# ViliamVadocz/takzero

Measured on AMD Instinct MI355X. Metric: mcts_simulations_per_s, higher is better.
Workload: dtype f16

## Files before the change

takzero_amd/build.py:

```python
import os
import subprocess
import sys

HERE = os.path.dirname(os.path.abspath(__file__))
CSRC = os.path.join(HERE, "csrc")
OUT = os.path.join(HERE, "libtakzero_hip.so")
ARCH = "gfx950"
UNITS = [
    ("tz_text.cpp", ["-ffp-contract=off"]),
    ("tz_ot.cpp", []),
    ("tz_host.cpp", ["-ffp-contract=off"]),
    ("tz_host_learn.cpp", ["-ffp-contract=off"]),
    ("tz_comm.cpp", []),
    ("tz_tree.hip", ["-ffp-contract=off", "-fhip-fp32-correctly-rounded-divide-sqrt"]),
    ("tz_capi.hip", ["-ffp-contract=off", "-fhip-fp32-correctly-rounded-divide-sqrt"]),
    ("tz_nn.hip", []),
    ("tz_nn_split.hip", []),
    ("tz_nn_c6.hip", []),
    ("tz_nn_c6b.hip", []),
    ("tz_nn_c6c.hip", []),
    ("tz_learn.hip", ["-ffp-contract=off"]),
]
COMMON = ["-O3", "-std=c++17", "-fPIC", "--offload-arch=" + ARCH, "-fno-fast-math", "-Wall", "-Wno-unused-function",
          "-Wno-unused-result"]


def _stale(target, deps):
    if not os.path.exists(target):
        return True
    t = os.path.getmtime(target)
    return any(os.path.getmtime(d) > t for d in deps)


def build(force=False, verbose=False, ablations=None):
    hipcc = os.environ.get("HIPCC", "/opt/rocm/bin/hipcc")
    if ablations is None:
        ablations = os.environ.get("TZ_BUILD_ABLATIONS", "0") not in ("", "0")
    stamp = os.path.join(CSRC, ".ablations")
    if ablations != os.path.exists(stamp):
        force_nn = True
        if ablations:
            open(stamp, "w").close()
        elif os.path.exists(stamp):
            os.remove(stamp)
    else:
        force_nn = False
    headers = [os.path.join(CSRC, f) for f in os.listdir(CSRC) if f.endswith(".h")]
    headers.append(os.path.join(os.path.dirname(HERE), "include", "takzero_hip.h"))
    objs = []
    procs = []
    for src, extra in UNITS:
        s = os.path.join(CSRC, src)
        o = os.path.join(CSRC, src.rsplit(".", 1)[0] + ".o")
        objs.append(o)
        nn = src in ("tz_nn.hip", "tz_nn_split.hip", "tz_nn_c6.hip", "tz_nn_c6b.hip", "tz_nn_c6c.hip")
        deps = [s] + headers + ([os.path.join(CSRC, "tz_nn.hip")] if nn else []) + ([os.path.join(CSRC, "tz_nn_c6.hip")] if src.startswith("tz_nn_c6") else [])
        if force or _stale(o, deps) or (force_nn and nn):
            cmd = [hipcc] + COMMON + extra + (["-DTZ_ABLATIONS"] if ablations and nn else []) + ["-x", "hip", "-c", s, "-o", o]
            if verbose:
                print(" ".join(cmd))
            procs.append((src, subprocess.Popen(cmd, stdout=subprocess.PIPE, stderr=subprocess.STDOUT)))
    failed = False
    for src, p in procs:
        out, _ = p.communicate()
        if p.returncode != 0:
            failed = True
            sys.stderr.write("---- %s ----\n%s\n" % (src, out.decode(errors="replace")))
        elif verbose and out:
            sys.stderr.write(out.decode(errors="replace"))
    if failed:
        raise RuntimeError("hipcc failed")
    if force or procs or _stale(OUT, objs):
        cmd = [hipcc, "-shared", "-fPIC", "--offload-arch=" + ARCH, "-o", OUT] + objs + ["-ldl"]
        subprocess.check_call(cmd)
    return OUT


if __name__ == "__main__":
    print(build(force="--force" in sys.argv, verbose=True, ablations=True if "--ablations" in sys.argv else None))
```

takzero_amd/csrc/tz_nn.hip:

```cpp
#include "tz_nn.h"
#include "tz_fp8.h"
#include "tz_fp6.h"
#include <type_traits>
#include "tz_ot.h"

#include <algorithm>
#include <cmath>
#include <cstdio>
#include <cstdlib>
#include <cstring>
#include <atomic>
#include <map>
#include <memory>
#include <mutex>
#include <thread>

int tz_nn_launch_split(int sp, int n, const void* net_args, int max_positions, hipStream_t st);
int tz_nn_launch_c6(int n, const void* net_args, int max_positions, hipStream_t st);
size_t tz_nn_c6_seed_bytes(int n, int max_positions);

namespace {

typedef float f32x4 __attribute__((ext_vector_type(4)));
typedef unsigned int u32x4 __attribute__((ext_vector_type(4)));
typedef __bf16 bf16x8 __attribute__((ext_vector_type(8)));
typedef __bf16 bf16x4 __attribute__((ext_vector_type(4)));
typedef _Float16 f16x8 __attribute__((ext_vector_type(8)));
typedef _Float16 f16x4 __attribute__((ext_vector_type(4)));

template <typename ET>
struct Elem;
template <>
struct Elem<__bf16> {
    typedef bf16x8 x8;
    typedef bf16x4 x4;
    static __device__ __forceinline__ f32x4 mfma(x8 a, x8 b, f32x4 c) { return __builtin_amdgcn_mfma_f32_16x16x32_bf16(a, b, c, 0, 0, 0); }
    static __device__ __forceinline__ __bf16 cvt(float x) { return (__bf16)x; }
    static __device__ __forceinline__ __bf16 relu_cvt(float x) { return (__bf16)(x > 0.f ? x : 0.f); }
};
template <>
struct Elem<_Float16> {
    typedef f16x8 x8;
    typedef f16x4 x4;
    static __device__ __forceinline__ f32x4 mfma(x8 a, x8 b, f32x4 c) { return __builtin_amdgcn_mfma_f32_16x16x32_f16(a, b, c, 0, 0, 0); }
    static __device__ __forceinline__ _Float16 cvt(float x) { return (_Float16)__builtin_amdgcn_fmed3f(x, -65504.0f, 65504.0f); }
    static __device__ __forceinline__ _Float16 relu_cvt(float x) { return (_Float16)__builtin_amdgcn_fmed3f(x, 0.0f, 65504.0f); }
};


constexpr int LDS_ROWB = 64;
constexpr int FILTERS = 256;
__device__ __forceinline__ int lds_piece(int row, int q) { return ((q + 2 * ((row >> 2) & 1)) & 3) << 4; }
template <int LAYOUT>
struct LdsImg {
    static constexpr int ROW_PAD = 528;
    __host__ __device__ static constexpr size_t bytes(int lrows) { return LAYOUT ? (size_t)lrows * LDS_ROWB * 8 : (size_t)lrows * ROW_PAD; }
    __device__ static __forceinline__ int store_addr(int row, int ci, int plane_bytes) {
        return LAYOUT ? (ci >> 2) * plane_bytes + row * LDS_ROWB + lds_piece(row, ci & 3) : row * ROW_PAD + ci * 16;
    }
    __device__ static __forceinline__ int read_base(bool ok, int v, int q, int zrow) {
        if (LAYOUT) {
            const int sr = ok ? v : zrow + (v & 7);
            return sr * LDS_ROWB + lds_piece(sr, q);
        }
        return (ok ? v : zrow) * ROW_PAD + q * 16;
    }
};

__host__ __device__ constexpr int c6_position_of(int c) {
    const int w = c >> 5, o = c & 31;
    return 32 * (4 * (w >> 2) + (o >> 3)) + 8 * (w & 3) + (o & 7);
}
__host__ __device__ constexpr int c6_channel_at(int pos) {
    const int plane = pos >> 5, piece = (pos >> 3) & 3, e = pos & 7;
    return 32 * (4 * (plane >> 2) + piece) + 8 * (plane & 3) + e;
}
static_assert(c6_channel_at(c6_position_of(77)) == 77 && c6_position_of(c6_channel_at(200)) == 200 && c6_position_of(32) == 8 && c6_position_of(8) == 32, "c6 channel places");

__host__ __device__ constexpr int ppt_for(int nb) { return nb == 1 ? 64 : nb == 3 ? 16 : nb == 4 ? 12 : nb == 5 ? 8 : 4; }

__device__ __forceinline__ void default_reserves_d(int n, int& stones, int& caps) {
    stones = n == 3 ? 10 : n == 4 ? 15 : n == 5 ? 21 : 30;
    caps = n >= 5 ? 1 : 0;
}

template <int NB>
__device__ __forceinline__ float plane_value(const tz_state* s, int px, int c, int flat_diff) {
    constexpr int SS = 3 + (NB - 1) + (NB + 1), NN = NB * NB;
    const int to_move = s->to_move;
    if (c < 2 * SS) {
        const int side = c / SS, k = c % SS;
        const int top = s->top[px], h = s->height[px];
        if (top == TZ_EMPTY) return 0.0f;
        const unsigned long long colors = s->colors[px];
        if (k < 3) {
            const int topc = (int)((colors >> (h - 1)) & 1ull);
            return (top == k + 1 && (topc != to_move) == (side == 1)) ? 1.0f : 0.0f;
        }
        const int idx = h - 2 - (k - 3);
        if (idx < 0) return 0.0f;
        const int color = (int)((colors >> idx) & 1ull);
        return ((color != to_move) == (side == 1)) ? 1.0f : 0.0f;
    }
    const int e = c - 2 * SS;
    int ds, dc;
    default_reserves_d(NB, ds, dc);
    const int mine = to_move, other = 1 - to_move;
    switch (e) {
        case 0: return (float)s->stones[mine] / (float)ds;
        case 1: return dc ? (float)s->caps[mine] / (float)dc : 0.0f;
        case 2: return (float)s->stones[other] / (float)ds;
        case 3: return dc ? (float)s->caps[other] / (float)dc : 0.0f;
        case 4: return to_move == 1 ? 1.0f : 0.0f;
        case 5: return ((float)flat_diff - (float)s->half_komi / 2.0f) / (float)NN;
        default: return 0.0f;
    }
}

template <int NB>
__device__ __forceinline__ int state_flat_diff(const tz_state* s) {
    int d = 0;
    for (int i = 0; i < NB * NB; i++) {
        if (s->top[i] == TZ_FLAT) {
            const int col = (int)((s->colors[i] >> (s->height[i] - 1)) & 1ull);
            d += col == 0 ? 1 : -1;
        }
    }
    return d;
}

struct ConvArgs {
    const void* in;
    const tz_state* states;
    const int32_t* game_index;
    const int32_t* count_dev;
    int count_host;
    const uint16_t* w;
    const float* bias;
    const void* residual;
    void* out;
    int cin_pad, kc_total, ct_total, out_stride, cin_real;
    int relu, out_f32, has_res;
    int in_stride;
    int groups;
    int in_z, w_z_frags, bias_z, out_z;
};

template <int NB, int RT, int TAPS, int LAYOUT>
__device__ __forceinline__ void tap_bases(const int (&yx)[RT], int tap, int lr, int q, int zrow, int (&abase)[RT]) {
    const int dy = TAPS == 9 ? tap / 3 - 1 : 0, dx = TAPS == 9 ? tap % 3 - 1 : 0;
#pragma unroll
    for (int rt = 0; rt < RT; rt++) {
        const int y = (yx[rt] & 0xff) + dy, x = (yx[rt] >> 8) + dx;
        const bool ok = y >= 0 && y < NB && x >= 0 && x < NB;
        abase[rt] = LdsImg<LAYOUT>::read_base(ok, rt * 16 + lr + dy * NB + dx, q, zrow);
    }
}

template <int NB, int RT, int TAPS, int LAYOUT>
__device__ __forceinline__ void tap_bases_rc(int tap, int lr, int q, int rows, int zrow, int (&abase)[RT]) {
    constexpr int NN = NB * NB;
    const int dy = TAPS == 9 ? tap / 3 - 1 : 0, dx = TAPS == 9 ? tap % 3 - 1 : 0;
#pragma unroll
    for (int rt = 0; rt < RT; rt++) {
        const int r = rt * 16 + lr, px = r % NN;
        const int y = px / NB + dy, x = px % NB + dx;
        const bool ok = r < rows && y >= 0 && y < NB && x >= 0 && x < NB;
        abase[rt] = LdsImg<LAYOUT>::read_base(ok, r + dy * NB + dx, q, zrow);
    }
}

template <int NB, int P, int RN, int TAPS, bool FROM_STATE, int ABL = 0, bool SINGLE = false, int NW = 8, int LAYOUT = 1, typename ET = __bf16, int OCC = 2>
__global__ __launch_bounds__(NW * 64, OCC) void conv_mfma_kernel(ConvArgs a) {
    typedef typename Elem<ET>::x8 ex8;
    typedef typename Elem<ET>::x4 ex4;
    constexpr int NT = NW * 64;
    constexpr int NN = NB * NB, ROWS = P * NN, RT = (ROWS + 15) / 16, LROWS = RT * 16 + 8, ZROW = RT * 16;
    constexpr int PLANE = LROWS * LDS_ROWB;
    constexpr int KSTEP = LAYOUT ? PLANE : 64;
    extern __shared__ __attribute__((aligned(16))) unsigned char lds[];
    const int count = a.count_dev ? *a.count_dev : a.count_host;
    const int pos0 = blockIdx.x * P;
    if (pos0 >= count) return;
    const int tid = threadIdx.x, lane = tid & 63;
    const int wave = __builtin_amdgcn_readfirstlane(tid >> 6);
    const int q = lane >> 4, lr = lane & 15;
    const int valid_rows = min(ROWS, (count - pos0) * NN);
    const size_t m0 = (size_t)pos0 * NN;
    const int ct0 = (blockIdx.y * NW + wave) * RN;
    const __amdgpu_buffer_rsrc_t wrsrc = __builtin_amdgcn_make_buffer_rsrc(
        const_cast<uint16_t*>(a.w), 0, (a.groups > 1 ? a.groups * a.w_z_frags : TAPS * a.kc_total * a.ct_total) * 1024, 0x00020000);
    const int lane16 = lane * 16;
    auto wload = [&](int tap, int kcg, int j) -> ex8 {
        const int frag = (int)blockIdx.z * a.w_z_frags + (tap * a.kc_total + kcg) * a.ct_total + (ct0 + j);
        const u32x4 r = __builtin_amdgcn_raw_buffer_load_b128(wrsrc, lane16, frag * 1024, 0);
        return __builtin_bit_cast(ex8, r);
    };
    f32x4 acc[RT][RN];

    if constexpr (SINGLE) {
        static_assert(!FROM_STATE, "SINGLE is for bf16 activations");
        {
            const uint16_t* in = reinterpret_cast<const uint16_t*>(a.in);
            constexpr int NLOAD = (LROWS * 32 + NT - 1) / NT;
            uint4 v[NLOAD];
#pragma unroll
            for (int i = 0; i < NLOAD; i++) {
                const int id = tid + i * NT, row = id >> 5, ci = id & 31;
                v[i] = make_uint4(0, 0, 0, 0);
                if (row < valid_rows) v[i] = *reinterpret_cast<const uint4*>(in + (m0 + row) * 256 + ci * 8);
            }
#pragma unroll
            for (int i = 0; i < NLOAD; i++) {
                const int id = tid + i * NT, row = id >> 5, ci = id & 31;
                if (row < LROWS) *reinterpret_cast<uint4*>(lds + LdsImg<LAYOUT>::store_addr(row, ci, PLANE)) = v[i];
            }
        }
        ex8 bq[4][RN];
#pragma unroll
        for (int j = 0; j < RN; j++) {
            bq[0][j] = wload(0, 0, j);
            bq[1][j] = wload(0, 1, j);
        }
        __syncthreads();
#pragma unroll
        for (int rt = 0; rt < RT; rt++)
#pragma unroll
            for (int j = 0; j < RN; j++) acc[rt][j] = f32x4{0.f, 0.f, 0.f, 0.f};
        int abase[RT];
        tap_bases_rc<NB, RT, TAPS, LAYOUT>(0, lr, q, ROWS, ZROW, abase);
        ex8 av[RT];
#pragma unroll
        for (int rt = 0; rt < RT; rt++) av[rt] = *reinterpret_cast<const ex8*>(lds + abase[rt]);
        for (int tap = 0; tap < TAPS; tap++) {
#pragma unroll
            for (int kc = 0; kc < 8; kc++) {
                if constexpr ((ABL & 2) == 0) {
                    if (kc + 2 < 8) {
#pragma unroll
                        for (int j = 0; j < RN; j++) bq[(kc + 2) & 3][j] = wload(tap, kc + 2, j);
                    } else if (tap + 1 < TAPS) {
#pragma unroll
                        for (int j = 0; j < RN; j++) bq[(kc + 2) & 3][j] = wload(tap + 1, kc + 2 - 8, j);
                    }
                    __builtin_amdgcn_sched_barrier(0);
                }
                if (kc == 7) {
                    int lr_t = lr;
                    asm volatile("" : "+v"(lr_t));
                    tap_bases_rc<NB, RT, TAPS, LAYOUT>(tap + 1 < TAPS ? tap + 1 : tap, lr_t, q, ROWS, ZROW, abase);
                }
                if (LAYOUT == 1 && kc == 4) {
#pragma unroll
                    for (int rt = 0; rt < RT; rt++) {
                        abase[rt] += 4 * PLANE;
                        asm volatile("" : "+v"(abase[rt]));
                    }
                }
#pragma unroll
                for (int rt = 0; rt < RT; rt++) {
#pragma unroll
                    for (int j = 0; j < RN; j++)
                        acc[rt][j] = Elem<ET>::mfma(bq[kc & 3][j], av[rt], acc[rt][j]);
                    if constexpr ((ABL & 1) == 0) {
                        if (kc < 7) av[rt] = *reinterpret_cast<const ex8*>(lds + abase[rt] + (kc + 1 - (LAYOUT == 1 && kc >= 4 ? 4 : 0)) * KSTEP);
                        else av[rt] = *reinterpret_cast<const ex8*>(lds + abase[rt]);
                    }
                }
            }
        }
    } else {
        int yx[RT];
#pragma unroll
        for (int rt = 0; rt < RT; rt++) {
            const int r = rt * 16 + lr, px = r % NN;
            yx[rt] = r < ROWS ? ((px / NB) | ((px % NB) << 8)) : 0x7f7f;
        }
#pragma unroll
        for (int rt = 0; rt < RT; rt++)
#pragma unroll
            for (int j = 0; j < RN; j++) acc[rt][j] = f32x4{0.f, 0.f, 0.f, 0.f};
        const int nslices = (a.cin_pad + 255) / 256;
        constexpr int NLOAD = FROM_STATE ? 1 : (LROWS * 32 + NT - 1) / NT;
        uint4 stage[NLOAD];
        auto fetch_slice = [&](int slice) {
            const int cpr_s = min(256, a.cin_pad - slice * 256) / 8;
            const uint16_t* in = reinterpret_cast<const uint16_t*>(a.in) + (size_t)blockIdx.z * a.in_z + slice * 256;
#pragma unroll
            for (int i = 0; i < NLOAD; i++) {
                const int id = tid + i * NT, row = id >> 5, ci = id & 31;
                stage[i] = make_uint4(0, 0, 0, 0);
                if (row < valid_rows && ci < cpr_s) stage[i] = *reinterpret_cast<const uint4*>(in + (m0 + row) * a.in_stride + ci * 8);
            }
        };
        if constexpr (!FROM_STATE) fetch_slice(0);
        for (int slice = 0; slice < nslices; slice++) {
            const int cs = min(256, a.cin_pad - slice * 256);
            const int kcs = cs / 32, cpr = cs / 8;
            __syncthreads();
            if constexpr (FROM_STATE) {
                for (int row = tid; row < LROWS; row += NT) {
                    const bool ok = row < valid_rows;
                    const tz_state* s = nullptr;
                    int px = 0, fd = 0;
                    if (ok) {
                        const int pos = pos0 + row / NN;
                        px = row % NN;
                        s = a.states + (a.game_index ? a.game_index[pos] : pos);
                        fd = state_flat_diff<NB>(s);
                    }
                    for (int c8 = 0; c8 < cpr; c8++) {
                        ex8 v;
#pragma unroll
                        for (int k = 0; k < 8; k++) {
                            const int c = c8 * 8 + k;
                            v[k] = (ET)((ok && c < a.cin_real) ? plane_value<NB>(s, px, c, fd) : 0.0f);
                        }
                        *reinterpret_cast<ex8*>(lds + LdsImg<LAYOUT>::store_addr(row, c8, PLANE)) = v;
                    }
                }
            } else {
#pragma unroll
// ... 2328 lines not shown
                                p8[at] = tz_f32_to_e4m3((wv - (float)hi) * 2048.0f * sw);
                                p8[at + 64 * 32] = tz_f32_to_e4m3((float)hi * sw);
                            }
                        }
            if ((rc = upload(p8, &L->w8))) return rc;
        }
        if (with_c6) {
            if (L->cin_pad % 128) return tz_fail(TZ_EINVAL, "weights: TZ_PREC_F16C6 needs input channels in multiples of 128");
            const int g_total = L->cin_pad / 128;
            constexpr size_t REC = 3328;
            std::vector<unsigned char> p6((size_t)taps * g_total * ct_total * REC, 0);
            for (int t = 0; t < taps; t++)
                for (int g = 0; g < g_total; g++)
                    for (int ct = 0; ct < ct_total; ct++) {
                        unsigned char* rec = p6.data() + (((size_t)t * g_total + g) * ct_total + ct) * REC;
                        for (int lane = 0; lane < 64; lane++) {
                            const int co = ct * 16 + (lane & 15), q = lane >> 4;
                            float lo[32], hi[32], amax_l = 0.0f, amax_h = 0.0f;
                            for (int i = 0; i < 32; i++) {
                                const int ci = 128 * g + 32 * (i >> 3) + 8 * q + (i & 7);
                                const float wv = (co < cout && ci < cin) ? W(co, ci, t) : 0.0f;
                                const _Float16 h = (_Float16)wv;
                                hi[i] = (float)h;
                                lo[i] = wv - (float)h;
                                amax_h = std::max(amax_h, fabsf(hi[i]));
                                amax_l = std::max(amax_l, fabsf(lo[i]));
                            }
                            const uint32_t bl = tz_e2m3_block_scale_byte(amax_l), bh = tz_e2m3_block_scale_byte(amax_h);
                            uint8_t cl[32], ch[32];
                            for (int i = 0; i < 32; i++) {
                                cl[i] = tz_f32_to_e2m3(ldexpf(lo[i], 127 - (int)bl));
                                ch[i] = tz_f32_to_e2m3(ldexpf(hi[i], 127 - (int)bh));
                            }
                            uint32_t sl[6], sh[6];
                            tz_pack_fp6x32(cl, sl);
                            tz_pack_fp6x32(ch, sh);
                            memcpy(rec + 0 * 1536 + lane * 16, sl, 16);
                            memcpy(rec + 0 * 1536 + 1024 + lane * 8, sl + 4, 8);
                            memcpy(rec + 1 * 1536 + lane * 16, sh, 16);
                            memcpy(rec + 1 * 1536 + 1024 + lane * 8, sh + 4, 8);
                            const uint32_t sw = bl | (bh << 8);
                            memcpy(rec + 3072 + lane * 4, &sw, 4);
                        }
                    }
            if ((rc = upload(p6, &L->w8))) return rc;
        }
        return upload(p, &L->w_mfma);
    }
    std::vector<float> f((size_t)taps * cin * cout);
    for (int t = 0; t < taps; t++)
        for (int ci = 0; ci < cin; ci++)
            for (int co = 0; co < cout; co++) f[((size_t)t * cin + ci) * cout + co] = W(co, ci, t);
    return upload(f, &L->w_f32);
}

void free_layer(ConvW* L) {
    if (L->w_mfma) (void)hipFree(L->w_mfma);
    if (L->w_lo) (void)hipFree(L->w_lo);
    if (L->w8) (void)hipFree(L->w8);
    if (L->w_f32) (void)hipFree(L->w_f32);
    if (L->bias) (void)hipFree(L->bias);
    *L = ConvW();
}

int bn_fold(const TensorMap& m, const std::string& p, int c, std::vector<float>& scale, std::vector<float>& bias) {
    std::vector<float> g, b, mean, var;
    int rc;
    if ((rc = get_tensor(m, p + ".weight", c, g))) return rc;
    if ((rc = get_tensor(m, p + ".bias", c, b))) return rc;
    if ((rc = get_tensor(m, p + ".running_mean", c, mean))) return rc;
    if ((rc = get_tensor(m, p + ".running_var", c, var))) return rc;
    scale.resize(c);
    bias.resize(c);
    for (int i = 0; i < c; i++) {
        const float s = g[i] / sqrtf(var[i] + 1e-5f);
        scale[i] = s;
        bias[i] = b[i] - mean[i] * s;
    }
    return TZ_OK;
}

struct NetWeights {
    ConvW conv_in, policy;
    std::vector<ConvW> res;
    uint16_t* tower_w = nullptr;
    uint16_t* tower_w_lo = nullptr;
    unsigned char* tower_w8 = nullptr;
    float* c8_scales = nullptr;
    float* tower_bias = nullptr;
    float* heads = nullptr;
    ConvW rnd[2][3];
    uint16_t* rndw[3] = {nullptr, nullptr, nullptr};
    float* rndb[3] = {nullptr, nullptr, nullptr};
    float rnd_min = 0.f, rnd_max = 1.f;
    float* simhash = nullptr;
};

void free_weights(NetWeights& w) {
    free_layer(&w.conv_in);
    free_layer(&w.policy);
    for (auto& l : w.res) free_layer(&l);
    w.res.clear();
    if (w.tower_w) (void)hipFree(w.tower_w);
    if (w.tower_w_lo) (void)hipFree(w.tower_w_lo);
    if (w.tower_w8) (void)hipFree(w.tower_w8);
    if (w.c8_scales) (void)hipFree(w.c8_scales);
    if (w.tower_bias) (void)hipFree(w.tower_bias);
    w.tower_w = nullptr;
    w.tower_w_lo = nullptr;
    w.tower_w8 = nullptr;
    w.c8_scales = nullptr;
    w.tower_bias = nullptr;
    if (w.heads) (void)hipFree(w.heads);
    w.heads = nullptr;
    for (int a = 0; a < 2; a++)
        for (int b = 0; b < 3; b++) free_layer(&w.rnd[a][b]);
    for (int l = 0; l < 3; l++) {
        if (w.rndw[l]) (void)hipFree(w.rndw[l]);
        if (w.rndb[l]) (void)hipFree(w.rndb[l]);
        w.rndw[l] = nullptr;
        w.rndb[l] = nullptr;
    }
    if (w.simhash) (void)hipFree(w.simhash);
    w.simhash = nullptr;
}

int build_weights(tz_net* net, const TensorMap& m, NetWeights& W) {
    const int nn = net->nn, cin = net->cin, prec = net->precision;
    std::vector<float> w, scale, bias;
    int rc;
    if ((rc = get_tensor(m, "core.input_conv2d.weight", (size_t)FILTERS * cin * 9, w))) return rc;
    if ((rc = bn_fold(m, "core.batch_norm", FILTERS, scale, bias))) return rc;
    const bool split = prec == TZ_PREC_F16X2, c8 = prec == TZ_PREC_F16C8, c6 = prec == TZ_PREC_F16C6;
    std::vector<int> c6_perm(FILTERS);
    for (int pos = 0; pos < FILTERS; pos++) c6_perm[pos] = c6_channel_at(pos);
    const std::vector<int>* tower_perm = c6 ? &c6_perm : nullptr;
    if ((rc = build_layer(prec, 9, cin, FILTERS, 256, w, scale, bias, nullptr, &W.conv_in, split || c8 || c6))) return rc;
    W.res.resize(2 * net->blocks);
    {
        const int nl = 2 * net->blocks;
        const int workers = std::max(1, std::min(nl, std::min(16, (int)std::thread::hardware_concurrency())));
        std::atomic<int> next{0}, failed{TZ_OK};
        std::string first_error;
        std::mutex mu;
        const bool background = g_upload_stream != nullptr;
        auto work = [&]() {
            if (hipSetDevice(net->device) != hipSuccess) {
                failed = TZ_EDEVICE;
                return;
            }
            std::unique_ptr<UploadStream> upload_stream(background ? new UploadStream() : nullptr);
            if (upload_stream && !upload_stream->mine) {
                std::lock_guard<std::mutex> lk(mu);
                if (failed == TZ_OK) {
                    failed = TZ_EDEVICE;
                    first_error = "weights: cannot create an upload stream for a build thread";
                }
                return;
            }
            std::vector<float> lw, lscale, lbias;
            for (int l = next++; l < nl && failed == TZ_OK; l = next++) {
                const std::string p = "core.res_block_" + std::to_string(l / 2) + ((l & 1) ? ".b" : ".a");
                int r = get_tensor(m, p + ".conv2d.weight", (size_t)FILTERS * FILTERS * 9, lw);
                if (!r) r = bn_fold(m, p + ".batch_norm", FILTERS, lscale, lbias);
                if (!r) r = build_layer(prec, 9, FILTERS, FILTERS, 256, lw, lscale, lbias, tower_perm, &W.res[l], split, c8, c6);
                if (r) {
                    std::lock_guard<std::mutex> lk(mu);
                    if (failed == TZ_OK) {
                        failed = r;
                        first_error = tz_last_error();
                    }
                }
            }
        };
        std::vector<std::thread> pool;
        for (int t = 1; t < workers; t++) pool.emplace_back(work);
        work();
        for (auto& t : pool) t.join();
        if (failed != TZ_OK) return tz_fail(failed, first_error.empty() ? "weights: a tower layer could not be built" : first_error);
    }
    if (prec != TZ_PREC_F32 && net->blocks > 0) {
        const size_t layer_elems = (size_t)9 * 8 * 16 * 64 * 8, nl = W.res.size();
        TZ_HIP(hipMalloc(&W.tower_w, nl * layer_elems * 2));
        if (split) TZ_HIP(hipMalloc(&W.tower_w_lo, nl * layer_elems * 2));
        const size_t layer_bytes8 = c6 ? (size_t)9 * 2 * 16 * 3328 : (size_t)9 * 2 * 16 * 2 * 64 * 32;
        if (c8 || c6) TZ_HIP(hipMalloc(&W.tower_w8, nl * layer_bytes8));
        TZ_HIP(hipMalloc(&W.tower_bias, nl * FILTERS * sizeof(float)));
        for (size_t l = 0; l < nl; l++) {
            if ((rc = copy_sync(W.tower_w + l * layer_elems, W.res[l].w_mfma, layer_elems * 2, hipMemcpyDeviceToDevice))) return rc;
            if (split && (rc = copy_sync(W.tower_w_lo + l * layer_elems, W.res[l].w_lo, layer_elems * 2, hipMemcpyDeviceToDevice))) return rc;
            if ((c8 || c6) && (rc = copy_sync(W.tower_w8 + l * layer_bytes8, W.res[l].w8, layer_bytes8, hipMemcpyDeviceToDevice))) return rc;
            if ((rc = copy_sync(W.tower_bias + l * FILTERS, W.res[l].bias, FILTERS * sizeof(float), hipMemcpyDeviceToDevice))) return rc;
        }
    }
    if ((rc = get_tensor(m, "policy.conv2d.weight", (size_t)net->pol_ch * FILTERS * 9, w))) return rc;
    if ((rc = get_tensor(m, "policy.conv2d.bias", net->pol_ch, bias))) return rc;
    if ((rc = build_layer(prec, 9, FILTERS, net->pol_ch, net->pol_stride, w, {}, bias, tower_perm, &W.policy, split, c8, c6))) return rc;
    if (c8) {
        std::vector<float> cs;
        for (auto& l : W.res) cs.push_back(l.c8_scale);
        cs.push_back(W.policy.c8_scale);
        if ((rc = upload(cs, &W.c8_scales))) return rc;
    }
    std::vector<float> hv, hu, lv, lu, t1;
    if ((rc = get_tensor(m, "value.conv2d.weight", FILTERS, hv))) return rc;
    if ((rc = get_tensor(m, "ube.conv2d.weight", FILTERS, hu))) return rc;
    if ((rc = get_tensor(m, "value.linear.weight", nn, lv))) return rc;
    if ((rc = get_tensor(m, "ube.linear.weight", nn, lu))) return rc;
    std::vector<float> hw;
    hw.insert(hw.end(), hv.begin(), hv.end());
    hw.insert(hw.end(), hu.begin(), hu.end());
    hw.insert(hw.end(), lv.begin(), lv.end());
    hw.insert(hw.end(), lu.begin(), lu.end());
    for (const char* nm : {"value.conv2d.bias", "ube.conv2d.bias", "value.linear.bias", "ube.linear.bias"}) {
        if ((rc = get_tensor(m, nm, 1, t1))) return rc;
        hw.push_back(t1[0]);
    }
    if ((rc = upload(hw, &W.heads))) return rc;
    if (net->has_rnd) {
        const int in_size = cin * nn;
        std::vector<int> perm(in_size);
        for (int px = 0; px < nn; px++)
            for (int c = 0; c < cin; c++) perm[px * cin + c] = c * nn + px;
        const char* nets[2] = {"rnd_learning", "rnd_target"};
        const char* layers[3] = {"input_linear", "hidden_linear", "final_linear"};
        const int dims[4] = {in_size, 1024, 1024, 512};
        for (int a = 0; a < 2; a++)
            for (int l = 0; l < 3; l++) {
                const std::string p = std::string(nets[a]) + "." + layers[l];
                if ((rc = get_tensor(m, p + ".weight", (size_t)dims[l + 1] * dims[l], w))) return rc;
                if ((rc = get_tensor(m, p + ".bias", dims[l + 1], bias))) return rc;
                if ((rc = build_layer(prec, 1, dims[l], dims[l + 1], 256, w, {}, bias, l == 0 ? &perm : nullptr, &W.rnd[a][l])))
                    return rc;
            }
        if (prec != TZ_PREC_F32) {
            std::vector<float> wa, wb, ba, bb;
            if ((rc = get_tensor(m, "rnd_learning.input_linear.weight", (size_t)1024 * in_size, wa))) return rc;
            if ((rc = get_tensor(m, "rnd_target.input_linear.weight", (size_t)1024 * in_size, wb))) return rc;
            if ((rc = get_tensor(m, "rnd_learning.input_linear.bias", 1024, ba))) return rc;
            if ((rc = get_tensor(m, "rnd_target.input_linear.bias", 1024, bb))) return rc;
            wa.insert(wa.end(), wb.begin(), wb.end());
            ba.insert(ba.end(), bb.begin(), bb.end());
            ConvW cat;
            if ((rc = build_layer(prec, 1, in_size, 2048, 256, wa, {}, ba, &perm, &cat))) return rc;
            W.rndw[0] = cat.w_mfma;
            W.rndb[0] = cat.bias;
            for (int l = 1; l < 3; l++) {
                const size_t welems = (size_t)(W.rnd[0][l].cin_pad / 32) * (W.rnd[0][l].cout_pad / 16) * 512;
                const size_t belems = W.rnd[0][l].cout_pad;
                TZ_HIP(hipMalloc(&W.rndw[l], 2 * welems * 2));
                TZ_HIP(hipMalloc(&W.rndb[l], 2 * belems * sizeof(float)));
                for (int a = 0; a < 2; a++) {
                    if ((rc = copy_sync(W.rndw[l] + a * welems, W.rnd[a][l].w_mfma, welems * 2, hipMemcpyDeviceToDevice))) return rc;
                    if ((rc = copy_sync(W.rndb[l] + a * belems, W.rnd[a][l].bias, belems * sizeof(float), hipMemcpyDeviceToDevice))) return rc;
                }
            }
        }
        if ((rc = get_tensor(m, "min", 1, t1))) return rc;
        W.rnd_min = t1[0];
        if ((rc = get_tensor(m, "max", 1, t1))) return rc;
        W.rnd_max = t1[0];
    }
    if (net->has_hash) {
        if ((rc = get_tensor(m, "simhash_matrix", (size_t)cin * nn * 32, w))) return rc;
        if ((rc = upload(w, &W.simhash))) return rc;
    }
    return TZ_OK;
}

__host__ __device__ constexpr int ppt_small(int nb) { return nb == 1 ? 64 : nb == 3 ? 7 : nb == 4 ? 6 : nb == 5 ? 4 : 3; }

int conv_cfg() {
    static int cfg = -1;
    if (cfg < 0) {
        const char* e = getenv("TZ_CONV_CFG");
        cfg = e ? atoi(e) : 0;
    }
    return cfg;
}

template <int NB, int P, int NW, int RN, int TAPS, bool FROM_STATE, bool SINGLE, int ABL = 0, int LAYOUT = 1, typename ET = __bf16, int OCC = 2>
int launch_conv(const ConvArgs& a, int max_positions, int n_blocks_y, hipStream_t st) {
    constexpr int NN = NB * NB, RT = (P * NN + 15) / 16, LROWS = RT * 16 + 8;
    const size_t smem = LdsImg<LAYOUT>::bytes(LROWS);
    auto kern = conv_mfma_kernel<NB, P, RN, TAPS, FROM_STATE, ABL, SINGLE, NW, LAYOUT, ET, OCC>;
    static bool attr_done[64] = {};
    int attr_dev = 0;
    TZ_HIP(hipGetDevice(&attr_dev));
    bool& attr_set = attr_done[attr_dev & 63];
    if (!attr_set) {
        TZ_HIP(hipFuncSetAttribute(reinterpret_cast<const void*>(kern), hipFuncAttributeMaxDynamicSharedMemorySize, (int)smem));
        attr_set = true;
    }
    dim3 grid((max_positions + P - 1) / P, n_blocks_y, a.groups > 1 ? a.groups : 1);
    hipLaunchKernelGGL(kern, grid, dim3(NW * 64), smem, st, a);
    hipError_t e = hipGetLastError();
    if (e != hipSuccess) return tz_fail(TZ_EDEVICE, std::string("conv launch: ") + hipGetErrorString(e));
    return TZ_OK;
}

int linear_grouped_bf16(int precision, const uint16_t* w, const float* bias, int groups, int cin_pad, int cout_pad, const void* in,
                        int in_stride, int in_z, void* out, int out_stride, int out_z, bool relu, bool out_f32,
                        const int32_t* count_dev, int count_host, int max_positions, hipStream_t st) {
    ConvArgs a;
    memset(&a, 0, sizeof a);
    a.in = in;
    a.count_dev = count_dev;
    a.count_host = count_host;
    a.w = w;
    a.bias = bias;
    a.out = out;
    a.cin_pad = cin_pad;
    a.kc_total = cin_pad / 32;
    a.ct_total = cout_pad / 16;
    a.out_stride = out_stride;
    a.cin_real = cin_pad;
    a.relu = relu;
    a.out_f32 = out_f32;
    a.in_stride = in_stride;
    a.groups = groups;
    a.in_z = in_z;
    a.w_z_frags = a.kc_total * a.ct_total;
    a.bias_z = cout_pad;
    a.out_z = out_z;
    if (max_positions <= 128) {
        if (prec_is_f16(precision)) return launch_conv<1, 32, 8, 2, 1, false, false, 0, 1, _Float16>(a, max_positions, cout_pad / 256, st);
        return launch_conv<1, 32, 8, 2, 1, false, false>(a, max_positions, cout_pad / 256, st);
    }
    if (prec_is_f16(precision)) return launch_conv<1, 128, 8, 2, 1, false, false, 0, 1, _Float16>(a, max_positions, cout_pad / 256, st);
    return launch_conv<1, 128, 8, 2, 1, false, false>(a, max_positions, cout_pad / 256, st);
}

template <int NB, typename ET>
int conv_board(const ConvArgs& a, int cout_pad, bool from_state, int max_positions, hipStream_t st) {
    constexpr int PA = ppt_for(NB), PB = ppt_small(NB);
    const bool wide = cout_pad % 256 == 0;
    const int by = wide ? cout_pad / 256 : cout_pad / 128;
    if (conv_cfg() == 0) {
        if (from_state) return launch_conv<NB, PA, 8, 2, 9, true, false, 0, 1, ET>(a, max_positions, by, st);
        if (wide) return launch_conv<NB, PA, 8, 2, 9, false, true, 0, 1, ET>(a, max_positions, by, st);
        return launch_conv<NB, PA, 8, 1, 9, false, true, 0, 1, ET>(a, max_positions, by, st);
    }
    if (from_state) return launch_conv<NB, PB, 4, 4, 9, true, false, 0, 1, ET>(a, max_positions, by, st);
    if (wide) return launch_conv<NB, PB, 4, 4, 9, false, true, 0, 1, ET>(a, max_positions, by, st);
    return launch_conv<NB, PB, 4, 2, 9, false, true, 0, 1, ET>(a, max_positions, by, st);
}

template <typename ET>
int conv_dispatch(int n, bool board, const ConvArgs& a, int cout_pad, bool from_state, int max_positions, hipStream_t st) {
    if (!board) return launch_conv<1, 64, 8, 2, 1, false, false, 0, 1, ET>(a, max_positions, cout_pad / 256, st);
    switch (n) {
        case 3: return conv_board<3, ET>(a, cout_pad, from_state, max_positions, st);
        case 4: return conv_board<4, ET>(a, cout_pad, from_state, max_positions, st);
        case 5: return conv_board<5, ET>(a, cout_pad, from_state, max_positions, st);
        case 6: return conv_board<6, ET>(a, cout_pad, from_state, max_positions, st);
    }
    return tz_fail(TZ_EINVAL, "conv: unsupported board size");
}

int conv_bf16(tz_net* net, const ConvW& L, const void* in, const tz_state* states, const int32_t* gidx,
              const int32_t* count_dev, int count_host, int max_positions, const void* residual, void* out,
              int out_stride, bool relu, bool out_f32, bool board, hipStream_t st) {
    ConvArgs a;
    a.in = in;
    a.states = states;
    a.game_index = gidx;
    a.count_dev = count_dev;
    a.count_host = count_host;
    a.w = L.w_mfma;
    a.bias = L.bias;
    a.residual = residual;
    a.out = out;
    a.cin_pad = L.cin_pad;
    a.kc_total = L.cin_pad / 32;
    a.ct_total = L.cout_pad / 16;
    a.out_stride = out_stride;
    a.cin_real = L.cin;
    a.relu = relu;
    a.out_f32 = out_f32;
    a.has_res = residual != nullptr;
    a.in_stride = L.cin_pad;
    a.groups = 1;
    a.in_z = a.w_z_frags = a.bias_z = a.out_z = 0;
    if (prec_is_f16(net->precision)) return conv_dispatch<_Float16>(net->n, board, a, L.cout_pad, in == nullptr, max_positions, st);
    return conv_dispatch<__bf16>(net->n, board, a, L.cout_pad, in == nullptr, max_positions, st);
}

#ifdef TZ_ABLATIONS
template <int NB>
int launch_tower4x2(const TowerArgs& a, int max_positions, hipStream_t st) {
    constexpr int P = ppt_for(NB), NN = NB * NB, RT = (P * NN + 15) / 16, LROWS = RT * 16 + 8;
    const size_t smem = (size_t)LROWS * LDS_ROWB * 8 + (size_t)9 * RT * 64 * 4;
    auto kern = tower4x2_mfma_kernel<NB, P>;
    static bool attr_done[64] = {};
    int attr_dev = 0;
    TZ_HIP(hipGetDevice(&attr_dev));
    bool& attr_set = attr_done[attr_dev & 63];
    if (!attr_set) {
        TZ_HIP(hipFuncSetAttribute(reinterpret_cast<const void*>(kern), hipFuncAttributeMaxDynamicSharedMemorySize, (int)smem));
        attr_set = true;
    }
    hipLaunchKernelGGL(kern, dim3((max_positions + P - 1) / P), dim3(512), smem, st, a);
    hipError_t e = hipGetLastError();
    if (e != hipSuccess) return tz_fail(TZ_EDEVICE, std::string("tower4x2 launch: ") + hipGetErrorString(e));
    return TZ_OK;
}
#endif

template <int NB, int OPT = 0, typename ET = __bf16>
int launch_tower(const TowerArgs& a, int max_positions, hipStream_t st) {
    constexpr int P = ppt_for(NB), NN = NB * NB, RT = (P * NN + 15) / 16, LROWS = RT * 16 + 8;
    const size_t smem = (size_t)LROWS * LDS_ROWB * 8 + ((OPT & 4096) ? (size_t)9 * RT * 64 * 4 : 0);
    auto kern = tower_mfma_kernel<NB, P, OPT, ET>;
    static bool attr_done[64] = {};
    int attr_dev = 0;
    TZ_HIP(hipGetDevice(&attr_dev));
    bool& attr_set = attr_done[attr_dev & 63];
    if (!attr_set) {
        TZ_HIP(hipFuncSetAttribute(reinterpret_cast<const void*>(kern), hipFuncAttributeMaxDynamicSharedMemorySize, (int)smem));
        attr_set = true;
    }
    hipLaunchKernelGGL(kern, dim3((max_positions + P - 1) / P), dim3(512), smem, st, a);
    hipError_t e = hipGetLastError();
    if (e != hipSuccess) return tz_fail(TZ_EDEVICE, std::string("tower launch: ") + hipGetErrorString(e));
    return TZ_OK;
}

int tower_bf16(tz_net* net, const void* in, void* out, const int32_t* count_dev, int count_host, int max_positions,
               hipStream_t st) {
    TowerArgs a;
    a.in = reinterpret_cast<const uint16_t*>(in);
    a.out = reinterpret_cast<uint16_t*>(out);
    a.w = net->tower_w;
    a.bias = net->tower_bias;
    a.count_dev = count_dev;
    a.count_host = count_host;
    a.nlayers = 2 * net->blocks;
    const bool h = prec_is_f16(net->precision);
    switch (net->n) {
        case 3: return h ? launch_tower<3, 4224, _Float16>(a, max_positions, st) : launch_tower<3, 4224>(a, max_positions, st);
        case 4: return h ? launch_tower<4, 4224, _Float16>(a, max_positions, st) : launch_tower<4, 4224>(a, max_positions, st);
        case 5: return h ? launch_tower<5, 4224, _Float16>(a, max_positions, st) : launch_tower<5, 4224>(a, max_positions, st);
        case 6: return h ? launch_tower<6, 4224, _Float16>(a, max_positions, st) : launch_tower<6, 4224>(a, max_positions, st);
    }
    return tz_fail(TZ_EINVAL, "tower: unsupported board size");
}

#endif

int net_fused_mode() {
    static int mode = -1;
    if (mode < 0) {
        const char* e = getenv("TZ_TOWER");
        mode = e ? atoi(e) : 2;
    }
    return mode;
}

constexpr int NET_SPLIT_MAX_GROUPS = 64;
constexpr size_t NET_SPLIT_PLANE_BYTES = 7680;
constexpr int NET_SPLIT_MAX_POSITIONS = 4 * NET_SPLIT_MAX_GROUPS;

template <int NB, int RNP, typename ET, bool PERM, int P = ppt_for(NB), int SP = 0, int ABL = 0, int TT = 0, int NW = 8, int SPLIT = 1>
int launch_net(const NetArgs& a, int max_positions, hipStream_t st) {
    constexpr int RT = RowMap<NB, P, PERM>::RT, LROWS = RT * 16 + 8;
    constexpr bool ROWTAB = SP != 0 && NB == 6 && P == 4;
    constexpr size_t tap_bytes = TT ? (size_t)9 * RT * RowMap<NB, P, PERM>::PPT * sizeof(int) : (size_t)9 * RT * 64 * (ROWTAB ? 1 : SP == 2 ? sizeof(uint16_t) : sizeof(int));
    constexpr size_t smem = (size_t)LROWS * LDS_ROWB * (SP == 2 ? (NB == 6 ? 16 : 20) : SP ? 16 : 8) + 2 * RT * 16 * sizeof(float) + tap_bytes + (SPLIT > 1 ? 16 : 0);
    static_assert(smem <= 160 * 1024, "net kernel: the LDS image does not fit a CU");
    auto kern = net_mfma_kernel<NB, P, RNP, ET, PERM, SP, ABL, TT, NW, SPLIT>;
    static bool attr_done[64] = {};
    int attr_dev = 0;
    TZ_HIP(hipGetDevice(&attr_dev));
    bool& attr_set = attr_done[attr_dev & 63];
    if (!attr_set) {
        TZ_HIP(hipFuncSetAttribute(reinterpret_cast<const void*>(kern), hipFuncAttributeMaxDynamicSharedMemorySize, (int)smem));
        attr_set = true;
    }
    int blocks = (max_positions + P - 1) / P;
    if (SPLIT > 1) {
        const int groups = (blocks + 7) / 8 * 8;
        if (groups > NET_SPLIT_MAX_GROUPS || !a.xch || !a.xch_count) return tz_fail(TZ_EINVAL, "net launch: the several-CU form is for small batches");
        TZ_HIP(hipMemsetAsync(a.xch_count, 0, (size_t)groups * 128, st));
        blocks = groups * SPLIT;
    }
    hipLaunchKernelGGL(kern, dim3(blocks), dim3(NW * 64), smem, st, a);
    hipError_t e = hipGetLastError();
    if (e != hipSuccess) return tz_fail(TZ_EDEVICE, std::string("net launch: ") + hipGetErrorString(e));
    return TZ_OK;
}

bool net_square_major() {
    static int v = -1;
    if (v < 0) {
        const char* e = getenv("TZ_NET_ROWS");
        v = (e && !strcmp(e, "board")) ? 0 : 1;
    }
    return v == 1;
}

int net_small_p(int max_positions) {
    static const bool full = getenv("TZ_NET_P") && !strcmp(getenv("TZ_NET_P"), "full");
    if (full) return 0;
    return max_positions <= 256 ? 1 : max_positions <= 512 ? 2 : max_positions <= 1024 ? 4 : 0;
}

#if defined(TZ_NN_C6_TU)
}
#elif defined(TZ_NN_SPLIT_TU)
}

int tz_nn_launch_split(int sp, int n, const void* net_args, int max_positions, hipStream_t st) {
    const NetArgs& a = *static_cast<const NetArgs*>(net_args);
    if (sp == 1) {
        if (n == 5 && a.xch && max_positions <= NET_SPLIT_MAX_POSITIONS) {
            if (max_positions <= NET_SPLIT_MAX_GROUPS) return launch_net<5, 1, _Float16, false, 1, 1, 0, 0, 4, 4>(a, max_positions, st);
            if (max_positions <= 2 * NET_SPLIT_MAX_GROUPS) return launch_net<5, 1, _Float16, false, 2, 1, 0, 0, 4, 4>(a, max_positions, st);
            return launch_net<5, 1, _Float16, false, 4, 1, 0, 0, 4, 4>(a, max_positions, st);
        }
        switch (n) {
            case 3: return launch_net<3, 1, _Float16, false, 8, 1>(a, max_positions, st);
            case 4: return launch_net<4, 1, _Float16, false, 6, 1>(a, max_positions, st);
            case 5: return launch_net<5, 1, _Float16, true, 4, 1>(a, max_positions, st);
            case 6:
                if (net_square_major() && max_positions >= 1024) return launch_net<6, 2, _Float16, true, 4, 1>(a, max_positions, st);
                return launch_net<6, 2, _Float16, false, 2, 1>(a, max_positions, st);
        }
        return tz_fail(TZ_EINVAL, "net: unsupported board size");
    }
#ifdef TZ_ABLATIONS
    if (n == 5 && getenv("TZ_NET_ABL") && atoi(getenv("TZ_NET_ABL")) == 16) return launch_net<5, 1, _Float16, true, 4, 2, 16>(a, max_positions, st);
    if (n == 5 && getenv("TZ_NET_ABL") && atoi(getenv("TZ_NET_ABL")) == 32) return launch_net<5, 1, _Float16, true, 4, 2, 32>(a, max_positions, st);
    if (n == 5 && getenv("TZ_NET_ABL") && atoi(getenv("TZ_NET_ABL")) == 48) return launch_net<5, 1, _Float16, true, 4, 2, 48>(a, max_positions, st);
#endif
    if (n == 5 && net_small_p(max_positions) == 1) return launch_net<5, 1, _Float16, false, 1, 2>(a, max_positions, st);
    if (n == 5 && net_small_p(max_positions) == 2) return launch_net<5, 1, _Float16, false, 2, 2>(a, max_positions, st);
    switch (n) {
        case 3: return launch_net<3, 1, _Float16, false, 8, 2>(a, max_positions, st);
        case 4: return launch_net<4, 1, _Float16, false, 6, 2>(a, max_positions, st);
        case 5: return launch_net<5, 1, _Float16, true, 4, 2>(a, max_positions, st);
        case 6:
            if (net_square_major() && max_positions >= 1024) return launch_net<6, 2, _Float16, true, 4, 2>(a, max_positions, st);
            return launch_net<6, 2, _Float16, false, 2, 2>(a, max_positions, st);
    }
    return tz_fail(TZ_EINVAL, "net: unsupported board size");
}
#else

bool net_p6_four() {
    static const bool four = getenv("TZ_NET_P6") && !strcmp(getenv("TZ_NET_P6"), "4");
    return four;
}

template <typename ET>
int net_fused_et(tz_net* net, const NetArgs& a, int max_positions, hipStream_t st) {
    const bool sq = net_square_major();
    const int small = net_small_p(max_positions);
    if (net->n == 5 && a.xch && max_positions <= NET_SPLIT_MAX_POSITIONS && sizeof(ET) == 2) {
        if (max_positions <= NET_SPLIT_MAX_GROUPS) return launch_net<5, 1, ET, false, 1, 0, 0, 0, 4, 4>(a, max_positions, st);
        if (max_positions <= 2 * NET_SPLIT_MAX_GROUPS) return launch_net<5, 1, ET, false, 2, 0, 0, 0, 4, 4>(a, max_positions, st);
        return launch_net<5, 1, ET, false, 4, 0, 0, 0, 4, 4>(a, max_positions, st);
    }
    if (net->n == 4 && a.xch && max_positions <= 2 * NET_SPLIT_MAX_GROUPS && sizeof(ET) == 2) {
        if (max_positions <= NET_SPLIT_MAX_GROUPS) return launch_net<4, 1, ET, false, 1, 0, 0, 0, 4, 4>(a, max_positions, st);
        return launch_net<4, 1, ET, false, 2, 0, 0, 0, 4, 4>(a, max_positions, st);
    }
    if (net->n == 6 && a.xch && max_positions <= 2 * NET_SPLIT_MAX_GROUPS && sizeof(ET) == 2) {
        if (max_positions <= NET_SPLIT_MAX_GROUPS) return launch_net<6, 2, ET, false, 1, 0, 0, 0, 4, 4>(a, max_positions, st);
        return launch_net<6, 2, ET, false, 2, 0, 0, 0, 4, 4>(a, max_positions, st);
    }
    if (net->n == 5 && small == 1) return launch_net<5, 1, ET, false, 1>(a, max_positions, st);
    if (net->n == 5 && small == 2) return launch_net<5, 1, ET, false, 2>(a, max_positions, st);
    if (net->n == 5 && small == 4) return launch_net<5, 1, ET, false, 4>(a, max_positions, st);
    if (net->n == 6 && small == 1) return launch_net<6, 2, ET, false, 1>(a, max_positions, st);
    if (net->n == 6 && small == 2) return launch_net<6, 2, ET, false, 2>(a, max_positions, st);
#ifdef TZ_ABLATIONS
    if (const char* e = getenv("TZ_NET_ABL")) {
        if (net->n == 5 && sq && small == 0 && sizeof(ET) == 2) {
            switch (atoi(e)) {
                case 1: return launch_net<5, 1, ET, true, 8, 0, 1>(a, max_positions, st);
                case 2: return launch_net<5, 1, ET, true, 8, 0, 2>(a, max_positions, st);
                case 3: return launch_net<5, 1, ET, true, 8, 0, 3>(a, max_positions, st);
                case 4: return launch_net<5, 1, ET, true, 8, 0, 4>(a, max_positions, st);
                case 8: return launch_net<5, 1, ET, true, 8, 0, 8>(a, max_positions, st);
                case 16: return launch_net<5, 1, ET, true, 8, 0, 16>(a, max_positions, st);
                case 32: return launch_net<5, 1, ET, true, 8, 0, 32>(a, max_positions, st);
                case 48: return launch_net<5, 1, ET, true, 8, 0, 48>(a, max_positions, st);
                case 64: return launch_net<5, 1, ET, true, 8, 0, 64>(a, max_positions, st);
                case 80: return launch_net<5, 1, ET, true, 8, 0, 80>(a, max_positions, st);
                default: break;
            }
        }
    }
#endif
    switch (net->n) {
        case 3: return sq ? launch_net<3, 1, ET, true>(a, max_positions, st) : launch_net<3, 1, ET, false>(a, max_positions, st);
        case 4: return launch_net<4, 1, ET, false>(a, max_positions, st);
        case 5:
#ifdef TZ_ABLATIONS
            if (sq && getenv("TZ_NET_TT") && atoi(getenv("TZ_NET_TT")) == 1) return launch_net<5, 1, ET, true, 8, 0, 0, 1>(a, max_positions, st);
#endif
#ifdef TZ_ABLATIONS
            if (sq && getenv("TZ_NET_W4") && atoi(getenv("TZ_NET_W4")) == 1) return launch_net<5, 1, ET, true, 8, 0, 0, 0, 4>(a, max_positions, st);
#endif
            return sq ? launch_net<5, 1, ET, true>(a, max_positions, st) : launch_net<5, 1, ET, false>(a, max_positions, st);
        case 6:
// ... 1220 lines not shown
```

Baseline: 1.486 million.

## Add pipelined MFMA GEMM kernel for large-batch grouped linear layers

Introduces a new dedicated GEMM kernel for grouped linear (MLP, likely RND) layers when the batch exceeds 128 positions, enabled by default. It double-buffers input slices in LDS with a swizzled layout and prefetches weight fragments through a register ring several K-steps ahead using buffer loads. The goal is to overlap global loads with MFMA work and get better reuse than the generic conv-based path. It needs K to be a multiple of 32 and N a multiple of 256, otherwise it returns an error, and it adds a separate code path to maintain.

```diff
diff --git a/takzero_amd/build.py b/takzero_amd/build.py
--- a/takzero_amd/build.py
+++ b/takzero_amd/build.py
@@ -19,6 +19,7 @@
     ("tz_nn_c6.hip", []),
     ("tz_nn_c6b.hip", []),
     ("tz_nn_c6c.hip", []),
+    ("tz_rnd.hip", []),
     ("tz_learn.hip", ["-ffp-contract=off"]),
 ]
 COMMON = ["-O3", "-std=c++17", "-fPIC", "--offload-arch=" + ARCH, "-fno-fast-math", "-Wall", "-Wno-unused-function",
diff --git a/takzero_amd/csrc/tz_nn.hip b/takzero_amd/csrc/tz_nn.hip
--- a/takzero_amd/csrc/tz_nn.hip
+++ b/takzero_amd/csrc/tz_nn.hip
@@ -18,6 +18,10 @@
 int tz_nn_launch_split(int sp, int n, const void* net_args, int max_positions, hipStream_t st);
 int tz_nn_launch_c6(int n, const void* net_args, int max_positions, hipStream_t st);
 size_t tz_nn_c6_seed_bytes(int n, int max_positions);
+bool tz_rnd_gemm_enabled();
+int tz_rnd_linear(bool f16, const uint16_t* w, const float* bias, int groups, int cin_pad, int cout_pad, const void* in, int in_stride, int in_z,
+                  void* out, int out_stride, int out_z, bool relu, bool out_f32, const int32_t* count_dev, int count_host, int max_positions,
+                  hipStream_t st);
 
 namespace {
 
@@ -2952,6 +2956,9 @@
 int linear_grouped_bf16(int precision, const uint16_t* w, const float* bias, int groups, int cin_pad, int cout_pad, const void* in,
                         int in_stride, int in_z, void* out, int out_stride, int out_z, bool relu, bool out_f32,
                         const int32_t* count_dev, int count_host, int max_positions, hipStream_t st) {
+    if (max_positions > 128 && tz_rnd_gemm_enabled())
+        return tz_rnd_linear(prec_is_f16(precision), w, bias, groups, cin_pad, cout_pad, in, in_stride, in_z, out, out_stride, out_z, relu, out_f32,
+                             count_dev, count_host, max_positions, st);
     ConvArgs a;
     memset(&a, 0, sizeof a);
     a.in = in;
diff --git a/takzero_amd/csrc/tz_rnd.hip b/takzero_amd/csrc/tz_rnd.hip
--- /dev/null
+++ b/takzero_amd/csrc/tz_rnd.hip
@@ -0,0 +1,222 @@
+#include "tz_nn.h"
+
+#include <cstdlib>
+#include <cstring>
+#include <string>
+
+namespace {
+
+typedef float f32x4 __attribute__((ext_vector_type(4)));
+typedef unsigned int u32x4 __attribute__((ext_vector_type(4)));
+typedef __bf16 bf16x8 __attribute__((ext_vector_type(8)));
+typedef __bf16 bf16x4 __attribute__((ext_vector_type(4)));
+typedef _Float16 f16x8 __attribute__((ext_vector_type(8)));
+typedef _Float16 f16x4 __attribute__((ext_vector_type(4)));
+
+template <typename ET>
+struct Elem;
+template <>
+struct Elem<__bf16> {
+    typedef bf16x8 x8;
+    typedef bf16x4 x4;
+    static __device__ __forceinline__ f32x4 mfma(x8 a, x8 b, f32x4 c) { return __builtin_amdgcn_mfma_f32_16x16x32_bf16(a, b, c, 0, 0, 0); }
+    static __device__ __forceinline__ __bf16 cvt(float x) { return (__bf16)x; }
+};
+template <>
+struct Elem<_Float16> {
+    typedef f16x8 x8;
+    typedef f16x4 x4;
+    static __device__ __forceinline__ f32x4 mfma(x8 a, x8 b, f32x4 c) { return __builtin_amdgcn_mfma_f32_16x16x32_f16(a, b, c, 0, 0, 0); }
+    static __device__ __forceinline__ _Float16 cvt(float x) { return (_Float16)__builtin_amdgcn_fmed3f(x, -65504.0f, 65504.0f); }
+};
+
+struct RndArgs {
+    const void* in;
+    const int32_t* count_dev;
+    int count_host;
+    const uint16_t* w;
+    const float* bias;
+    void* out;
+    int cin_pad, kc_total, ct_total, w_frags;
+    int in_stride, out_stride;
+    int in_z, w_z_frags, bias_z, out_z;
+    int relu, out_f32;
+};
+
+constexpr int RND_NW = 8, RND_NT = RND_NW * 64, RND_RN = 2;
+constexpr int RND_RING = 4, RND_AHEAD = 3;
+constexpr int RND_STORE_KC = 5;
+static_assert(RND_AHEAD < RND_RING && RND_STORE_KC < 7, "the ring slot being filled and the image being stored must be idle");
+
+__device__ __forceinline__ int rnd_piece(int row, int q) { return ((q + 2 * ((row >> 2) & 1)) & 3) << 4; }
+
+template <typename ET, int RT>
+__global__ __launch_bounds__(RND_NT, 2) void rnd_gemm_kernel(RndArgs a) {
+    typedef typename Elem<ET>::x8 ex8;
+    typedef typename Elem<ET>::x4 ex4;
+    constexpr int ROWS = RT * 16, PLANE = ROWS * 64, IMG = 8 * PLANE, NLOAD = ROWS * 32 / RND_NT;
+    static_assert(ROWS * 32 % RND_NT == 0 && 7 * PLANE < 65536, "tile loader / ds_read immediates");
+    extern __shared__ __attribute__((aligned(16))) unsigned char lds[];
+    const int count = a.count_dev ? *a.count_dev : a.count_host;
+    const int pos0 = blockIdx.x * ROWS;
+    if (pos0 >= count) return;
+    const int tid = threadIdx.x, lane = tid & 63;
+    const int wave = __builtin_amdgcn_readfirstlane(tid >> 6);
+    const int q = lane >> 4, lr = lane & 15;
+    const int valid_rows = min(ROWS, count - pos0);
+    const int ct0 = (blockIdx.y * RND_NW + wave) * RND_RN;
+    const int kc_total = a.kc_total, nslices = (a.cin_pad + 255) / 256;
+    const __amdgpu_buffer_rsrc_t wrsrc = __builtin_amdgcn_make_buffer_rsrc(const_cast<uint16_t*>(a.w), 0, a.w_frags * 1024, 0x00020000);
+    const int lane16 = lane * 16;
+    const int wfrag0 = (int)blockIdx.z * a.w_z_frags + ct0;
+    auto wload = [&](int g, int j) -> ex8 {
+        const int frag = wfrag0 + min(g, kc_total - 1) * a.ct_total + j;
+        const u32x4 r = __builtin_amdgcn_raw_buffer_load_b128(wrsrc, lane16, frag * 1024, 0);
+        return __builtin_bit_cast(ex8, r);
+    };
+    const size_t in0 = (size_t)blockIdx.z * a.in_z + (size_t)pos0 * a.in_stride;
+    const __amdgpu_buffer_rsrc_t irsrc = __builtin_amdgcn_make_buffer_rsrc(
+        const_cast<uint16_t*>(reinterpret_cast<const uint16_t*>(a.in) + in0), 0, ((valid_rows - 1) * a.in_stride + a.cin_pad) * 2, 0x00020000);
+    constexpr int OUTSIDE = (int)0x80000000u;
+    u32x4 stage[NLOAD];
+    auto fetch_slice = [&](int slice) {
+        const int cpr_s = max(0, min(256, a.cin_pad - slice * 256)) / 8;
+#pragma unroll
+        for (int i = 0; i < NLOAD; i++) {
+            const int id = tid + i * RND_NT, row = id >> 5, ci = id & 31;
+            stage[i] = __builtin_amdgcn_raw_buffer_load_b128(irsrc, ci < cpr_s ? (row * a.in_stride + ci * 8) * 2 : OUTSIDE, min(slice, nslices - 1) * 512, 0);
+        }
+    };
+    auto store_slice = [&](int img) {
+#pragma unroll
+        for (int i = 0; i < NLOAD; i++) {
+            const int id = tid + i * RND_NT, row = id >> 5, ci = id & 31;
+            *reinterpret_cast<u32x4*>(lds + img * IMG + (ci >> 2) * PLANE + row * 64 + rnd_piece(row, ci & 3)) = stage[i];
+        }
+    };
+
+    ex8 bq[RND_RING][RND_RN];
+    fetch_slice(0);
+#pragma unroll
+    for (int g = 0; g < RND_AHEAD; g++)
+#pragma unroll
+        for (int j = 0; j < RND_RN; j++) bq[g][j] = wload(g, j);
+    store_slice(0);
+    f32x4 acc[RT][RND_RN];
+#pragma unroll
+    for (int rt = 0; rt < RT; rt++)
+#pragma unroll
+        for (int j = 0; j < RND_RN; j++) acc[rt][j] = f32x4{0.f, 0.f, 0.f, 0.f};
+    int abase[RT];
+#pragma unroll
+    for (int rt = 0; rt < RT; rt++) abase[rt] = (rt * 16 + lr) * 64 + rnd_piece(rt * 16 + lr, q);
+    __syncthreads();
+    ex8 av[RT];
+#pragma unroll
+    for (int rt = 0; rt < RT; rt++) av[rt] = *reinterpret_cast<const ex8*>(lds + abase[rt]);
+
+    for (int slice = 0; slice < nslices; slice++) {
+        const int cur = (slice & 1) * IMG, nxt = IMG - cur;
+#pragma unroll
+        for (int kc = 0; kc < 8; kc++) {
+            const int g = slice * 8 + kc;
+            if (g >= kc_total) break;
+#pragma unroll
+            for (int j = 0; j < RND_RN; j++) bq[(kc + RND_AHEAD) % RND_RING][j] = wload(g + RND_AHEAD, j);
+            if (kc == 0) fetch_slice(slice + 1);
+            __builtin_amdgcn_sched_barrier(0);
+            if (kc == RND_STORE_KC) store_slice((slice + 1) & 1);
+            if (kc == 7) __syncthreads();
+#pragma unroll
+            for (int rt = 0; rt < RT; rt++) {
+#pragma unroll
+                for (int j = 0; j < RND_RN; j++) acc[rt][j] = Elem<ET>::mfma(bq[kc % RND_RING][j], av[rt], acc[rt][j]);
+                av[rt] = *reinterpret_cast<const ex8*>(lds + (kc < 7 ? cur + (kc + 1) * PLANE : nxt) + abase[rt]);
+            }
+        }
+    }
+
+#pragma unroll
+    for (int j = 0; j < RND_RN; j++) {
+        const int cbase = (ct0 + j) * 16 + q * 4;
+        const f32x4 bias = *reinterpret_cast<const f32x4*>(a.bias + (size_t)blockIdx.z * a.bias_z + cbase);
+#pragma unroll
+        for (int rt = 0; rt < RT; rt++) {
+            const int r = rt * 16 + lr;
+            if (r >= valid_rows) continue;
+            f32x4 v = acc[rt][j] + bias;
+            const size_t o = (size_t)blockIdx.z * a.out_z + (size_t)(pos0 + r) * a.out_stride + cbase;
+            if (a.relu) {
+#pragma unroll
+                for (int k = 0; k < 4; k++) v[k] = v[k] > 0.f ? v[k] : 0.f;
+            }
+            if (a.out_f32) {
+                *reinterpret_cast<f32x4*>(reinterpret_cast<float*>(a.out) + o) = v;
+            } else {
+                ex4 ov;
+#pragma unroll
+                for (int k = 0; k < 4; k++) ov[k] = Elem<ET>::cvt(v[k]);
+                *reinterpret_cast<ex4*>(reinterpret_cast<uint16_t*>(a.out) + o) = ov;
+            }
+        }
+    }
+}
+
+template <typename ET, int RT>
+int launch_rnd_gemm(const RndArgs& a, int groups, int cout_pad, int max_positions, hipStream_t st) {
+    constexpr int ROWS = RT * 16;
+    constexpr size_t smem = (size_t)2 * 8 * ROWS * 64;
+    auto kern = rnd_gemm_kernel<ET, RT>;
+    static bool attr_done[64] = {};
+    int dev = 0;
+    TZ_HIP(hipGetDevice(&dev));
+    if (!attr_done[dev & 63]) {
+        TZ_HIP(hipFuncSetAttribute(reinterpret_cast<const void*>(kern), hipFuncAttributeMaxDynamicSharedMemorySize, (int)smem));
+        attr_done[dev & 63] = true;
+    }
+    dim3 grid((max_positions + ROWS - 1) / ROWS, cout_pad / 256, groups);
+    hipLaunchKernelGGL(kern, grid, dim3(RND_NT), smem, st, a);
+    hipError_t e = hipGetLastError();
+    if (e != hipSuccess) return tz_fail(TZ_EDEVICE, std::string("rnd gemm launch: ") + hipGetErrorString(e));
+    return TZ_OK;
+}
+
+}
+
+bool tz_rnd_gemm_enabled() {
+    static const bool layers = [] {
+        const char* e = getenv("TZ_RND_MLP");
+        return e && !strcmp(e, "layers");
+    }();
+    return !layers;
+}
+
+int tz_rnd_linear(bool f16, const uint16_t* w, const float* bias, int groups, int cin_pad, int cout_pad, const void* in, int in_stride,
+                  int in_z, void* out, int out_stride, int out_z, bool relu, bool out_f32, const int32_t* count_dev, int count_host,
+                  int max_positions, hipStream_t st) {
+    if (cin_pad % 32 || cout_pad % 256 || in_stride % 8 || in_z % 8 || groups < 1)
+        return tz_fail(TZ_EINVAL, "rnd gemm: K must be a multiple of 32, N of 256, input rows 16-byte aligned");
+    RndArgs a;
+    memset(&a, 0, sizeof a);
+    a.in = in;
+    a.count_dev = count_dev;
+    a.count_host = count_host;
+    a.w = w;
+    a.bias = bias;
+    a.out = out;
+    a.cin_pad = cin_pad;
+    a.kc_total = cin_pad / 32;
+    a.ct_total = cout_pad / 16;
+    a.w_z_frags = a.kc_total * a.ct_total;
+    a.w_frags = groups * a.w_z_frags;
+    a.in_stride = in_stride;
+    a.out_stride = out_stride;
+    a.in_z = in_z;
+    a.bias_z = cout_pad;
+    a.out_z = out_z;
+    a.relu = relu;
+    a.out_f32 = out_f32;
+    const bool rows64 = cout_pad * groups < 2048;
+    if (f16) return rows64 ? launch_rnd_gemm<_Float16, 4>(a, groups, cout_pad, max_positions, st) : launch_rnd_gemm<_Float16, 8>(a, groups, cout_pad, max_positions, st);
+    return rows64 ? launch_rnd_gemm<__bf16, 4>(a, groups, cout_pad, max_positions, st) : launch_rnd_gemm<__bf16, 8>(a, groups, cout_pad, max_positions, st);
+}
```

After: 1.495 million (median of 6 runs). About the same (+0.6%).
